# infancy/ky

Measured on AMD Instinct MI355X. Metric: Msamples/s (paths*spp), higher is better.
Workload: dtype f32

## Files before the change

### include/kyhip.h

```cpp
#ifndef KYHIP_H
#define KYHIP_H

#ifndef __HIPCC_RTC__
#include <stddef.h>
#include <stdint.h>
#endif

#ifdef __cplusplus
extern "C" {
#endif

#define KYHIP_ABI_VERSION 4


typedef enum ky_shape_kind {
    KY_SHAPE_DISK      = 0,
    KY_SHAPE_TRIANGLE  = 1,
    KY_SHAPE_RECTANGLE = 2,
    KY_SHAPE_SPHERE    = 3
} ky_shape_kind;

typedef struct ky_shape {
    int32_t kind;
    float   p[4][3];
// ... 102 lines not shown
    int32_t  tile_first, tile_step;
} ky_render_params;

typedef enum ky_status {
    KY_OK                = 0,
    KY_ERR_INVALID_VALUE = -1,
    KY_ERR_LIMIT         = -2,
    KY_ERR_DEVICE        = -3,
    KY_ERR_NO_DEVICE     = -4
} ky_status;

const char* kyhip_last_error(void);
int         kyhip_set_engine(int engine);
int         kyhip_set_specialisation(int on);
int         kyhip_set_boxes(int on);
int         kyhip_set_shadow_queue(int mode);
int         kyhip_set_jit(int mode);
const char* kyhip_jit_status(void);
int         kyhip_jit_failures(void);
int64_t     kyhip_jit_compile(const char* name_expression);
uint64_t    kyhip_kernel_source_hash(void);
int         kyhip_abi_version(void);
int         kyhip_device_count(void);

int64_t kyhip_shard_tile_count(const ky_render_params* params);
int64_t kyhip_shard_float_count(const ky_render_params* params);
int64_t kyhip_film_term_limit(const ky_render_params* params, int n_lights, int engine, int deferred, float* limit);

int kyhip_render(int device, const ky_scene* scene, const ky_render_params* params,
                 float* film_rgb, size_t film_row_stride_px);
// ... 61 lines not shown

int kyhip_kat_intersect(int device, const ky_shape* shape, const float* rays7, int n, float* out8);

int kyhip_kat_camera(int device, const ky_camera* camera, const float* p_film2, int n, float* out6);

int kyhip_kat_bsdf(int device, const ky_material* material, const float* in12, int n, float* out13);

int kyhip_kat_light(int device, const ky_scene* scene, int light, const float* in11, int n, float* out11);

int kyhip_kat_scene_intersect(int device, const ky_scene* scene, const float* rays7, int n, float* out9);
int kyhip_kat_occluded(int device, const ky_scene* scene, const float* in9, int n, float* out1);
int kyhip_kat_any_pair(int device, const ky_scene* scene, const float* in13, int n, float* out2);
int kyhip_kat_occluded_between(int device, const ky_scene* scene, int light, const float* in9, int n, float* out1);
int kyhip_scene_non_occluders(const ky_scene* scene, int light, int* left_out, int n);
int kyhip_scene_boxes(const ky_scene* scene, int* box_face, int n);
int kyhip_scene_facts(const ky_scene* scene);

int kyhip_kat_li(int device, const ky_scene* scene, const ky_render_params* params,
                 int x, int y, int s0, int n, float* out3);

int kyhip_kat_nee(int device, const ky_scene* scene, int direct_sample, int light, const float* in15, int n, float* out6);
int kyhip_kat_single_light(int device, const ky_scene* scene, const float* in16, int n, float* out6);

int kyhip_kat_li_trace(int device, const ky_scene* scene, const ky_render_params* params, int x, int y, int s,
                       float* rows26, int max_rows, float* li3);

enum ky_smallpt_refl { KY_SP_DIFF = 0, KY_SP_SPEC = 1, KY_SP_REFR = 2 };

typedef struct ky_smallpt_sphere {
    double rad;
// ... 29 lines not shown
```

### ky_amd/_abi.py

```python
import ctypes as C
import os

_HERE = os.path.dirname(os.path.abspath(__file__))
LIB_DIR = os.path.join(_HERE, "lib")
REPO_ROOT = os.path.dirname(_HERE)

SHAPE_DISK, SHAPE_TRIANGLE, SHAPE_RECTANGLE, SHAPE_SPHERE = 0, 1, 2, 3
MATERIAL_MATTE, MATERIAL_MIRROR, MATERIAL_GLASS, MATERIAL_PLASTIC = 0, 1, 2, 3
LIGHT_POINT, LIGHT_DIRECTION, LIGHT_AREA, LIGHT_ENVIRONMENT = 0, 1, 2, 3
INTEGRATOR_POSITION, INTEGRATOR_NORMAL, INTEGRATOR_BASECOLOR = 0, 1, 2
INTEGRATOR_DIRECT_LIGHTING, INTEGRATOR_PATH_TRACING_ITERATION = 6, 11
INTEGRATOR_SIMPLE_PATH_TRACING_RECURSION, INTEGRATOR_PATH_TRACING_RECURSION, INTEGRATOR_PATH_TRACING_RECURSION_DEFERED = 8, 9, 10
DIRECT_IDLE, DIRECT_BSDF, DIRECT_LIGHT, DIRECT_BSDF_MIS, DIRECT_LIGHT_MIS, DIRECT_BOTH_MIS = 0, 4, 8, 16, 32, 48
DIRECT_SINGLE_LIGHT, DIRECT_SINGLE_BOTH_MIS = 1, 49
SAMPLER_DEBUG, SAMPLER_RANDOM = 0, 1
LIGHTING_EMIT, LIGHTING_DIRECT, LIGHTING_INDIRECT, LIGHTING_ALL = 1, 2, 4, 7
SP_VARIANT_SMALLPT, SP_VARIANT_REWRITE = 0, 1
KY_OK, KY_ERR_INVALID_VALUE, KY_ERR_LIMIT, KY_ERR_DEVICE, KY_ERR_NO_DEVICE = 0, -1, -2, -3, -4
MAX_SHAPES, MAX_SURFACES, MAX_MATERIALS, MAX_LIGHTS = 256, 256, 64, 16

CB_LIGHT_AREA, CB_LIGHT_DIRECTION, CB_LIGHT_POINT, CB_LIGHT_ENVIRONMENT = 1, 2, 4, 8
CB_LARGE_MIRROR, CB_LARGE_GLASS, CB_SMALL_MIRROR, CB_SMALL_GLASS = 16, 32, 64, 128
CB_BOTH_SMALL_SPHERES = CB_SMALL_MIRROR | CB_SMALL_GLASS
CB_DEFAULT_SCENE = CB_BOTH_SMALL_SPHERES | CB_LIGHT_AREA
# ... 58 lines not shown

class SmallptParams(C.Structure):
    _fields_ = [("width", C.c_int), ("height", C.c_int), ("samps", C.c_int), ("seed", C.c_uint32), ("max_depth", C.c_int),
                ("variant", C.c_int)]


SP_DIFF, SP_SPEC, SP_REFR = 0, 1, 2
SSP = C.POINTER(SmallptSphere)
SPP = C.POINTER(SmallptParams)

KYHIP_SYMBOLS = {
    "kyhip_last_error": (C.c_char_p, []),
    "kyhip_set_engine": (C.c_int, [C.c_int]),
    "kyhip_set_specialisation": (C.c_int, [C.c_int]),
    "kyhip_set_boxes": (C.c_int, [C.c_int]),
    "kyhip_set_shadow_queue": (C.c_int, [C.c_int]),
    "kyhip_set_jit": (C.c_int, [C.c_int]),
    "kyhip_jit_status": (C.c_char_p, []),
    "kyhip_jit_failures": (C.c_int, []),
    "kyhip_multi_status": (C.c_char_p, [C.c_int]),
    "kyhip_film_alloc": (C.c_void_p, [C.c_size_t]),
    "kyhip_film_free": (None, [C.c_void_p]),
    "kyhip_seam_threads": (C.c_int, []),
    "kyhip_jit_compile": (C.c_int64, [C.c_char_p]),
    "kyhip_kernel_source_hash": (C.c_uint64, []),
    "kyhip_abi_version": (C.c_int, []),
    "kyhip_device_count": (C.c_int, []),
    "kyhip_shard_tile_count": (C.c_int64, [PP]),
    "kyhip_shard_float_count": (C.c_int64, [PP]),
    "kyhip_film_term_limit": (C.c_int64, [PP, C.c_int, C.c_int, C.c_int, C.POINTER(C.c_float)]),
# ... 35 lines not shown
    "kyhip_kat_li_trace": (C.c_int, [C.c_int, SP, PP, C.c_int, C.c_int, C.c_int, C.c_void_p, C.c_int, C.c_void_p]),
    "kyhip_smallpt_scene": (C.c_int, [SSP]),
    "kyhip_smallpt_scene_rewrite": (C.c_int, [SSP]),
    "kyhip_smallpt_render": (C.c_int, [C.c_int, SSP, C.c_int, SPP, C.c_void_p]),
    "kyhip_smallpt_kat_radiance": (C.c_int, [C.c_int, SSP, C.c_int, SPP, C.c_int, C.c_int, C.c_int, C.c_int, C.c_int, C.c_int, C.c_void_p]),
    "kyhip_kat_intersect": (C.c_int, [C.c_int, C.POINTER(Shape), C.c_void_p, C.c_int, C.c_void_p]),
    "kyhip_kat_camera": (C.c_int, [C.c_int, C.POINTER(Camera), C.c_void_p, C.c_int, C.c_void_p]),
    "kyhip_kat_bsdf": (C.c_int, [C.c_int, C.POINTER(Material), C.c_void_p, C.c_int, C.c_void_p]),
    "kyhip_kat_light": (C.c_int, [C.c_int, SP, C.c_int, C.c_void_p, C.c_int, C.c_void_p]),
    "kyhip_kat_scene_intersect": (C.c_int, [C.c_int, SP, C.c_void_p, C.c_int, C.c_void_p]),
    "kyhip_kat_occluded": (C.c_int, [C.c_int, SP, C.c_void_p, C.c_int, C.c_void_p]),
    "kyhip_kat_any_pair": (C.c_int, [C.c_int, SP, C.c_void_p, C.c_int, C.c_void_p]),
    "kyhip_kat_occluded_between": (C.c_int, [C.c_int, SP, C.c_int, C.c_void_p, C.c_int, C.c_void_p]),
    "kyhip_scene_non_occluders": (C.c_int, [SP, C.c_int, C.c_void_p, C.c_int]),
    "kyhip_scene_boxes": (C.c_int, [SP, C.c_void_p, C.c_int]),
    "kyhip_scene_facts": (C.c_int, [SP]),
    "kyhip_kat_li": (C.c_int, [C.c_int, SP, PP, C.c_int, C.c_int, C.c_int, C.c_int, C.c_void_p]),
}

KYHOST_SYMBOLS = {
    "kyhost_last_error": (C.c_char_p, []),
    "kyhost_scene_create_cornell_box": (C.c_void_p, [C.c_int, C.c_float, C.c_float]),
    "kyhost_scene_create_mis": (C.c_void_p, [C.c_float, C.c_float]),
    "kyhost_scene_destroy": (None, [C.c_void_p]),
    "kyhost_scene_flatten": (SP, [C.c_void_p]),
    "kyhost_render": (C.c_int, [C.c_void_p, C.c_int, C.c_int, C.c_int, C.c_int, C.c_int, C.c_uint, C.c_int, C.c_int,
                                C.c_int, C.c_int, C.c_int, C.c_void_p, C.c_int]),
    "kyhost_render_lighting": (C.c_int, [C.c_void_p, C.c_int, C.c_int, C.c_int, C.c_int, C.c_int, C.c_uint, C.c_int, C.c_int,
                                         C.c_int, C.c_int, C.c_int, C.c_void_p, C.c_int, C.c_int]),
    "kyhost_debug_area": (C.c_int, [C.c_void_p, C.c_int, C.c_int, C.c_int, C.c_int, C.c_int, C.c_uint, C.c_int, C.c_int,
# ... 101 lines not shown
```

### ky_amd/api.py

```python
import ctypes as C

import numpy as np

from . import _abi as A


class KyError(RuntimeError):
    pass


def _check(rc, lib=None):
    if rc != A.KY_OK:
        lib = lib or A.load_kyhip()
        raise KyError(f"kyhip error {rc}: {lib.kyhip_last_error().decode()}")


def _fptr(a):
    assert a.dtype == np.float32 and a.flags["C_CONTIGUOUS"]
    return a.ctypes.data_as(C.c_void_p)


class SceneHandle:

    def __init__(self, ptr):
# ... 382 lines not shown
    if rc < 0:
        _check(rc)
    return rc


def scene_boxes(scene):
    lib = A.load_kyhip()
    n = _scene_ptr(scene).contents.surface_count
    out = np.zeros(max(1, n), np.int32)
    rc = lib.kyhip_scene_boxes(_scene_ptr(scene), out.ctypes.data_as(C.c_void_p), n)
    if rc < 0:
        _check(rc)
    return rc, out[:n].copy()


def kat_li(scene, params, x, y, s0, n, device=0):
    lib = A.load_kyhip()
    out = np.zeros((n, 3), np.float32)
    _check(lib.kyhip_kat_li(device, _scene_ptr(scene), C.byref(params), x, y, s0, n, _fptr(out)))
    return out


def kat_li_lighting(scene, params, lighting, x, y, s0, n, device=0):
    lib = A.load_kyhip()
    out = np.zeros((n, 3), np.float32)
    _check(lib.kyhip_kat_li_lighting(device, _scene_ptr(scene), C.byref(params), int(lighting), x, y, s0, n, _fptr(out)))
    return out


def kat_nee(scene, direct_sample, light, in15, device=0):
# ... 66 lines not shown
```

### ky_amd/csrc/ky_host.hpp

```cpp
#pragma once
#include <cstddef>
#include <cstdint>
#include <condition_variable>
#include <functional>
#include <mutex>
#include <string>
#include <utility>
#include <vector>
#include <sys/types.h>

#include "ky_shard.hpp"

namespace kyh {
using namespace kyd;

int fail(int code, const char* fmt, ...) __attribute__((format(printf, 2, 3)));
const std::string& last_error();

bool valid_params(const ky_render_params* p);
bool shard_in_range(const ky_render_params* p);
ShardConst make_shard(const ky_render_params* p);
RenderConst make_rc(const ky_render_params* p);
long long film_term_count(const ky_render_params* p, int n_lights, bool queue_engine, bool deferred);
float film_term_limit(long long n_terms);
// ... 29 lines not shown
struct NonOccluders {
    std::vector<char> wall;
    std::vector<char> light_ok;
    bool deferred_ok = false;
    int ts_light = -1;
    double ts_plane[4] = {0, 0, 0, 0};
    std::vector<char> ts_behind;
};
void find_non_occluders(const ky_scene* in, NonOccluders& R);
struct Boxes {
    struct Box { float lo[3], hi[3]; int face[6]; };
    std::vector<Box> box;
    std::vector<int> box_of;
};
void find_boxes(const ky_scene* in, Boxes& B);
int pack_scene(const ky_scene* in, DScene* out);
uint64_t scene_hash(const DScene& s);
bool scene_input(const ky_scene* in, std::vector<unsigned char>& out, uint64_t& hash);

constexpr int KY_SP_MAX_SPHERES = 32;
int smallpt_check(const ky_smallpt_sphere* spheres, int n, const ky_smallpt_params* p);

bool specialisation_enabled();
bool boxes_enabled();
int shadow_queue_mode();
bool shadow_queue_wanted(const ky_scene* scene);
int blocks_per_cu_cap();
enum { KY_ENGINE_LANE = 0, KY_ENGINE_QUEUE = 1 };
int current_engine();

int cpus_granted();
int seam_threads();
void host_add_rows(float* __restrict__ film, size_t stride_px, const float* __restrict__ src, int width, int y0, int y1);
class HostPool {
public:
    void run(int n, const std::function<void(int)>& fn);
private:
    void loop(int id);
    std::mutex job_m_, m_;
// ... 27 lines not shown
```

### ky_amd/csrc/ky_hostcheck.cpp

```cpp
#include <atomic>
#include <cstdlib>
#include <cstring>
#include <memory>
#include <thread>
#include <sys/wait.h>
#include <unistd.h>

#include "ky_blocks.hpp"
#include "ky_host.hpp"
#include "ky_noise.hpp"

using namespace kyh;

extern "C" {

int kyhostcheck_pack(const ky_scene* scene, int* feat, uint64_t* packed_hash, uint64_t* input_hash, int* n_planar_occ, int* ts_light) {
    std::unique_ptr<DScene> d(new DScene);
    const int rc = pack_scene(scene, d.get());
    if (rc != KY_OK) return rc;
    if (feat) *feat = d->feat;
    if (packed_hash) *packed_hash = scene_hash(*d);
    std::vector<unsigned char> in;
    uint64_t h = 0;
    const bool keyed = scene_input(scene, in, h);
// ... 178 lines not shown
        if (init) s = inside > 0 ? BlockState{-1, 0} : BlockState{0, 0};
        if (map && s.retired_at < 0) {
            int counted = 0, above = 0;
            for (int lane = 0; lane < KY_BLOCK_PIXELS; ++lane) {
                const int i = pixel_of_block(sh, b, lane);
                const int c = cls ? cls[i] : (pixel_inside(sh, i, p->width, p->height) ? kyn::KY_NOISE_INSIDE : kyn::KY_NOISE_PADDING);
                counted += c == kyn::KY_NOISE_INSIDE;
                above += c == kyn::KY_NOISE_INSIDE && map[i] > threshold;
            }
            if (block_retires(batches, min_batches, above, counted, max_fraction_above)) s = BlockState{front, batches};
        }
        state[2 * b] = s.retired_at; state[2 * b + 1] = s.batches;
    }
    if (!trailer) return KY_OK;
    return block_trailer_check(trailer, trailer_bytes, trailer_offset, sh.n_blocks, p->samples_per_pixel, samples_done, noise_batches);
}

static int no_gpu() { return fail(KY_ERR_NO_DEVICE, "sanitizer build of the host-only code: no GPU entry points"); }
int kyhip_device_count(void) { return 0; }
int kyhip_render(int, const ky_scene*, const ky_render_params* p, float*, size_t) { return valid_params(p) ? no_gpu() : fail(KY_ERR_INVALID_VALUE, "invalid render params"); }
int kyhip_render_multi(const int*, int, const ky_scene*, const ky_render_params* p, float*, size_t) { return valid_params(p) ? no_gpu() : fail(KY_ERR_INVALID_VALUE, "invalid render params"); }
int kyhip_render_tiles_device(int, const ky_scene*, const ky_render_params* p, float*, void*, size_t, void*) { return valid_params(p) ? no_gpu() : fail(KY_ERR_INVALID_VALUE, "invalid render params"); }
int kyhip_film_add_tiles_device(int, const ky_render_params*, const float*, float*, size_t, void*) { return no_gpu(); }
int kyhip_film_add_gathered_device(int, const ky_render_params*, int, const float*, size_t, float*, size_t, void*) { return no_gpu(); }
float kyhip_kernel_ms(int) { return -1.f; }
const char* kyhip_last_kernel(int) { return ""; }
const char* kyhip_multi_status(int) { return ""; }
void* kyhip_film_alloc(size_t) { return nullptr; }
void kyhip_film_free(void*) {}
int kyhip_kat_intersect(int, const ky_shape*, const float*, int, float*) { return no_gpu(); }
// ... 77 lines not shown
```

### ky_amd/csrc/ky_pack.cpp

```cpp
#include <algorithm>
#include <cmath>
#include <cstdarg>
#include <cstdio>
#include <cstdlib>
#include <cstring>
#include <limits>
#include <thread>
#include <sched.h>
#include <unistd.h>

#include "ky_blocks.hpp"
#include "ky_host.hpp"
#include "ky_noise.hpp"

namespace kyh {

static thread_local std::string g_error;

int fail(int code, const char* fmt, ...) {
    char buf[512];
    va_list ap;
    va_start(ap, fmt);
    vsnprintf(buf, sizeof buf, fmt, ap);
    va_end(ap);
// ... 523 lines not shown
        const char* e = std::getenv("KYHIP_SPECIALISE");
        g_specialise = (e && std::atoi(e) == 0) ? 0 : 1;
    }
    return g_specialise != 0;
}

static int g_boxes = -1;
bool boxes_enabled() {
    if (g_boxes < 0) {
        const char* e = std::getenv("KYHIP_BOXES");
        g_boxes = (e && std::atoi(e) == 0) ? 0 : 1;
    }
    return g_boxes != 0;
}

int pack_scene(const ky_scene* in, DScene* out) {
    if (!in) return fail(KY_ERR_INVALID_VALUE, "scene is NULL");
    if (in->surface_count < 0 || in->shape_count < 0 || in->material_count < 0 || in->light_count < 0)
        return fail(KY_ERR_INVALID_VALUE, "negative count in scene");
    if (in->surface_count > KYHIP_MAX_SURFACES || in->shape_count > KYHIP_MAX_SHAPES || in->material_count > KYHIP_MAX_MATERIALS ||
        in->light_count > KYHIP_MAX_LIGHTS)
        return fail(KY_ERR_LIMIT, "scene exceeds device limits (%d surfaces, %d shapes, %d materials, %d lights)", in->surface_count,
                    in->shape_count, in->material_count, in->light_count);
    if (in->environment_light < -1 || in->environment_light >= in->light_count) return fail(KY_ERR_INVALID_VALUE, "environment_light out of range");
    std::memset(out, 0, sizeof *out);
    out->n_surfaces = in->surface_count; out->n_lights = in->light_count; out->n_materials = in->material_count;
    out->env_light = in->environment_light;
    cp3(out->cam_position, in->camera.position); cp3(out->cam_front, in->camera.front); cp3(out->cam_right, in->camera.right);
    cp3(out->cam_up, in->camera.up);
    out->cam_inv_w = 1.f / in->camera.resolution[0]; out->cam_inv_h = 1.f / in->camera.resolution[1];
// ... 87 lines not shown
            }
            if (!fits) continue;
            DBox& d = BT.box[BT.n_box++];
            d.q0 = make_float4(b.lo[0], b.lo[1], b.lo[2], 0.f);
            d.q1 = make_float4(b.hi[0], b.hi[1], b.hi[2], 0.f);
            std::memcpy(&d.q0.w, &tag[0], 4); std::memcpy(&d.q1.w, &tag[1], 4);
            std::memcpy(&d.q2.x, &tag[2], 4); std::memcpy(&d.q2.y, &tag[3], 4); std::memcpy(&d.q2.z, &tag[4], 4); std::memcpy(&d.q2.w, &tag[5], 4);
            for (int f = 0; f < 6; ++f) if (b.face[f] >= 0) boxed[b.face[f]] = 1;
        }
        for (const PlanarEntry& e : planar)
            if (e.axis >= 0 && !boxed[e.surface]) { BT.n_aar_axis[e.axis]++; BT.aar[BT.n_aar++] = e.aar; }
        if (BT.n_aar > 0) BT.aar[BT.n_aar] = BT.aar[BT.n_aar - 1];
    }
    out->occ_deferred_ok = non.deferred_ok ? 1 : 0;
    out->ts_light = non.ts_light;
    out->feat = 0;
    if (specialisation_enabled()) {
        if (in->light_count == 1 && in->lights[0].kind == KY_LIGHT_AREA && in->environment_light < 0) out->feat |= KY_FEAT_SINGLE_AREA;
        if (in->light_count == 1 && (in->lights[0].kind == KY_LIGHT_POINT || in->lights[0].kind == KY_LIGHT_DIRECTION) && in->environment_light < 0)
            out->feat |= KY_FEAT_SINGLE_DELTA;
        if (in->light_count == 1 && in->lights[0].kind == KY_LIGHT_ENVIRONMENT && in->environment_light == 0) out->feat |= KY_FEAT_SINGLE_ENV;
        bool rect = true;
        for (int i = 0; i < in->light_count; ++i)
            if (in->lights[i].kind == KY_LIGHT_AREA) rect = rect && in->shapes[in->lights[i].shape].kind == KY_SHAPE_RECTANGLE;
        if (rect) out->feat |= KY_FEAT_RECT_LIGHTS;
        bool spheres = in->light_count > 0 && in->environment_light < 0;
        for (int i = 0; i < in->light_count; ++i)
            spheres = spheres && in->lights[i].kind == KY_LIGHT_AREA && in->shapes[in->lights[i].shape].kind == KY_SHAPE_SPHERE;
        for (int i = 0; i < in->surface_count; ++i)
            if (in->surfaces[i].area_light >= 0) spheres = spheres && in->shapes[in->surfaces[i].shape].kind == KY_SHAPE_SPHERE;
// ... 134 lines not shown
    uint64_t h0 = 0x9E3779B97F4A7C15ull, h1 = 0xC2B2AE3D27D4EB4Full;
    for (size_t i = 0; i + 1 < sizeof(DScene) / 8; i += 2) {
        h0 = (h0 ^ w[i]) * 0xff51afd7ed558ccdull; h0 ^= h0 >> 29;
        h1 = (h1 ^ w[i + 1]) * 0xc4ceb9fe1a85ec53ull; h1 ^= h1 >> 31;
    }
    if ((sizeof(DScene) / 8) & 1) h0 = (h0 ^ w[sizeof(DScene) / 8 - 1]) * 0xff51afd7ed558ccdull;
    return h0 ^ (h1 * 0x9E3779B97F4A7C15ull);
}

bool scene_input(const ky_scene* in, std::vector<unsigned char>& out, uint64_t& hash) {
    out.clear();
    if (!in || in->surface_count < 0 || in->shape_count < 0 || in->material_count < 0 || in->light_count < 0 || in->surface_count > KYHIP_MAX_SURFACES ||
        in->shape_count > KYHIP_MAX_SHAPES || in->material_count > KYHIP_MAX_MATERIALS || in->light_count > KYHIP_MAX_LIGHTS)
        return false;
    auto put = [&](const void* p, size_t n) { const unsigned char* b = (const unsigned char*)p; out.insert(out.end(), b, b + n); };
    const int32_t head[6] = {in->shape_count, in->material_count, in->light_count, in->surface_count, in->environment_light, (specialisation_enabled() ? 1 : 0) | (boxes_enabled() ? 2 : 0)};
    put(head, sizeof head);
    put(&in->camera, sizeof in->camera);
    if (in->shape_count) put(in->shapes, sizeof(ky_shape) * (size_t)in->shape_count);
    if (in->material_count) put(in->materials, sizeof(ky_material) * (size_t)in->material_count);
    if (in->light_count) put(in->lights, sizeof(ky_light) * (size_t)in->light_count);
    if (in->surface_count) put(in->surfaces, sizeof(ky_surface) * (size_t)in->surface_count);
    out.resize((out.size() + 7) & ~(size_t)7, 0);
    uint64_t h = 0x9E3779B97F4A7C15ull;
    for (size_t i = 0; i < out.size(); i += 8) {
        uint64_t w;
        std::memcpy(&w, &out[i], 8);
        h = (h ^ w) * 0xff51afd7ed558ccdull;
        h ^= h >> 29;
    }
    hash = h;
// ... 79 lines not shown

int smallpt_check(const ky_smallpt_sphere* spheres, int n, const ky_smallpt_params* p) {
    if (!spheres || !p) return fail(KY_ERR_INVALID_VALUE, "null argument");
    if (p->variant != KY_SP_VARIANT_SMALLPT && p->variant != KY_SP_VARIANT_REWRITE) return fail(KY_ERR_INVALID_VALUE, "unknown smallpt variant %d", p->variant);
    if (n <= 0 || n > KY_SP_MAX_SPHERES) return fail(KY_ERR_INVALID_VALUE, "1..%d spheres", KY_SP_MAX_SPHERES);
    if (p->width <= 0 || p->height <= 0 || p->width > 16384 || p->height > 16384 || p->samps <= 0 || p->max_depth < 0)
        return fail(KY_ERR_INVALID_VALUE, "invalid smallpt params");
    for (int i = 0; i < n; ++i)
        if (spheres[i].refl < KY_SP_DIFF || spheres[i].refl > KY_SP_REFR || !(spheres[i].rad > 0)) return fail(KY_ERR_INVALID_VALUE, "sphere %d is invalid", i);
    return KY_OK;
}

void set_engine_raw(int v) { g_engine = v; }
void set_specialise_raw(int v) { g_specialise = v; }
void set_boxes_raw(int v) { g_boxes = v; }
void set_shadow_queue_raw(int v) { g_shadow_queue = v; }
}

using namespace kyh;

extern "C" {

const char* kyhip_last_error(void) { return kyh::last_error().c_str(); }
int kyhip_seam_threads(void) { return kyh::seam_threads(); }
int kyhip_abi_version(void) { return KYHIP_ABI_VERSION; }


int kyhip_set_engine(int engine) {
    const int prev = current_engine();
    if (engine == KY_ENGINE_LANE || engine == KY_ENGINE_QUEUE) kyh::set_engine_raw(engine);
    return prev;
}
int kyhip_set_specialisation(int on) {
    const int prev = specialisation_enabled() ? 1 : 0;
    if (on == 0 || on == 1) kyh::set_specialise_raw(on);
    return prev;
}
int kyhip_set_boxes(int on) {
    const int prev = boxes_enabled() ? 1 : 0;
    if (on == 0 || on == 1) kyh::set_boxes_raw(on);
    return prev;
}
int kyhip_set_shadow_queue(int mode) {
    const int prev = shadow_queue_mode();
    if (mode >= -1 && mode <= 1) kyh::set_shadow_queue_raw(mode);
    return prev;
}

int kyhip_lighting_check(int integrator, int lighting) { return lighting_check(integrator, lighting); }
int kyhip_lighting_plan(const ky_render_params* p, int lighting, int* effective_depth, int* dropped) {
    LightingPlan pl;
    const int rc = lighting_plan(p, lighting, &pl);
    if (rc != KY_OK) return rc;
    if (effective_depth) *effective_depth = pl.effective_depth;
    if (dropped) *dropped = pl.dropped;
// ... 60 lines not shown
    const int rc = pack_scene(scene, &packed[0]);
    if (rc != KY_OK) return rc;
    if (n < scene->surface_count) return fail(KY_ERR_INVALID_VALUE, "box_face holds %d entries, the scene has %d surfaces", n, scene->surface_count);
    for (int i = 0; i < scene->surface_count; ++i) box_face[i] = -1;
    const DScene& P = packed[0];
    for (int b = 0; b < P.boxtrav.n_box; ++b) {
        const DBox& d = P.boxtrav.box[b];
        const float* src[6] = {&d.q0.w, &d.q1.w, &d.q2.x, &d.q2.y, &d.q2.z, &d.q2.w};
        for (int f = 0; f < 6; ++f) {
            uint32_t sidx;
            std::memcpy(&sidx, src[f], 4);
            if (sidx != (uint32_t)KY_BOX_NO_FACE) box_face[P.orig[sidx]] = 8 * b + f;
        }
    }
    return P.boxtrav.n_box;
}

int kyhip_smallpt_scene(ky_smallpt_sphere* out) {
    if (!out) return fail(KY_ERR_INVALID_VALUE, "null output");
    struct Row { double rad, p[3], e[3], c[3]; int refl; };
    static const Row rows[9] = {
        {1e5, {1e5 + 1, 40.8, 81.6}, {0, 0, 0}, {.75, .25, .25}, KY_SP_DIFF},
        {1e5, {-1e5 + 99, 40.8, 81.6}, {0, 0, 0}, {.25, .25, .75}, KY_SP_DIFF},
        {1e5, {50, 40.8, 1e5}, {0, 0, 0}, {.75, .75, .75}, KY_SP_DIFF},
        {1e5, {50, 40.8, -1e5 + 170}, {0, 0, 0}, {0, 0, 0}, KY_SP_DIFF},
        {1e5, {50, 1e5, 81.6}, {0, 0, 0}, {.75, .75, .75}, KY_SP_DIFF},
        {1e5, {50, -1e5 + 81.6, 81.6}, {0, 0, 0}, {.75, .75, .75}, KY_SP_DIFF},
        {16.5, {27, 16.5, 47}, {0, 0, 0}, {1 * .999, 1 * .999, 1 * .999}, KY_SP_SPEC},
        {16.5, {73, 16.5, 78}, {0, 0, 0}, {1 * .999, 1 * .999, 1 * .999}, KY_SP_REFR},
        {600, {50, 681.6 - .27, 81.6}, {12, 12, 12}, {0, 0, 0}, KY_SP_DIFF}};
// ... 19 lines not shown
```

### ky_amd/csrc/ky_render.hpp

```cpp
#pragma once
#include "ky_device.hpp"
#include "ky_shard.hpp"

using namespace kyd;

#ifndef KY_MAX_RETRACE
#define KY_MAX_RETRACE 1
#endif
#ifndef KY_REFILL_BATCH
#define KY_REFILL_BATCH 6
#endif
#ifndef KY_REFILL_WAIT
#define KY_REFILL_WAIT 4
#endif
#ifndef KY_RETRACE_THRESHOLD
#define KY_RETRACE_THRESHOLD 80
#endif
#ifndef KY_WAVES_PER_EU
#define KY_WAVES_PER_EU 7
#endif
#ifndef KY_WAVES_PER_EU_QUEUE
#define KY_WAVES_PER_EU_QUEUE 6
#endif
#ifndef KY_WAVES_PER_EU_QUEUE_FEAT
// ... 119 lines not shown
            const int n_need = __popcll(need_mask);
            while (!exhausted && cursor + n_need > fetched * 64) {
                unsigned id = blockIdx.x * 4u + (threadIdx.x >> 6);
                if (fetched > 0 && lane == 0) id = atomicAdd(counter, 1u) + gridDim.x * 4u;
                id = __builtin_amdgcn_readfirstlane(id);
                if (id >= sh.n_items) { exhausted = true; break; }
                const int c = (int)(id / (unsigned)sh.n_blocks) + sh.chunk_first;
                int b = (int)(id % (unsigned)sh.n_blocks);
                if constexpr (LISTED) {
                    typedef const int __attribute__((address_space(4))) * LiveList;
                    b = __builtin_amdgcn_readfirstlane(((LiveList)(const int*)(flags + sh.n_pix))[b]);
                }
                const int k = b / sh.blocks_per_tile, inner = b % sh.blocks_per_tile;
                const int bx = inner % sh.blocks_w, by = inner / sh.blocks_w;
                const int tile = sh.tile_first + k * sh.tile_step;
                if (lane == 0) {
                    ItemSlot it;
                    const int trow = tile / sh.tiles_x, tcol = (tile % sh.tiles_x + trow) % sh.tiles_x;
                    it.x0 = tcol * sh.tile_w + bx * 8;
                    it.y0 = trow * sh.tile_h + by * 8;
                    it.pix0 = (k * sh.tile_h + by * 8) * sh.tile_w + bx * 8;
                    chunk_range(chunk_plan(rc.spp), c, it.s_begin, it.s_end);
                    my_ring[fetched % KY_RING] = it;
                }
                ++fetched;
            }
            __builtin_amdgcn_fence(__ATOMIC_ACQ_REL, "wavefront");
            if (need) {
                const int mine = cursor + (int)__builtin_amdgcn_mbcnt_hi((unsigned)(need_mask >> 32), __builtin_amdgcn_mbcnt_lo((unsigned)need_mask, 0u));
                if (mine < fetched * 64) {
                    const ItemSlot it = my_ring[(mine >> 6) % KY_RING];
                    const int px = mine & 7, py = (mine >> 3) & 7;
                    const int x = it.x0 + px, y = it.y0 + py;
                    const bool in_range = x < rc.width && y < rc.height;
                    c_xy[tid] = x | (y << 16);
                    c_pix[tid] = it.pix0 + py * sh.tile_w + px;
                    if (!QUEUE) c_key[tid] = sampler_pixel_key(rc.seed, (uint32_t)(y * rc.width + x));
                    c_se[tid] = ((unsigned)it.s_begin << 7) | (unsigned)(it.s_end - it.s_begin);
// ... 79 lines not shown
```

### ky_amd/csrc/ky_scene.hpp

```cpp
#pragma once
#ifndef __HIPCC_RTC__
#include <hip/hip_vector_types.h>
#include <stdint.h>
#endif

#include "../../include/kyhip.h"

#if defined(__HIPCC__) || defined(__HIPCC_RTC__)
#define KY_HD __host__ __device__
#else
#define KY_HD
#endif

namespace kyd {

enum : int {
    TK_DISK = KY_SHAPE_DISK,
    TK_TRIANGLE = KY_SHAPE_TRIANGLE,
    TK_QUAD = KY_SHAPE_RECTANGLE,
    TK_SPHERE = KY_SHAPE_SPHERE,
    TK_PARALLELOGRAM = 4
};

struct DSurf {
// ... 47 lines not shown
    float e1[3];
    float inv_area;
    float n[3];
    int32_t n_carriers;
    int32_t carrier[4];
    int32_t sampled_is_surface;
    int32_t occ_ok;
    int32_t pdf_from_carrier;
    int32_t shadow_table;
    float aar[5];
    int32_t aar_axis;
    int32_t pad_a[2];
    DSurf isect;
};
constexpr int KY_MAX_CARRIERS = 4;
static_assert(sizeof(DLight) % 16 == 0 && __builtin_offsetof(DLight, p1) % 16 == 0 && __builtin_offsetof(DLight, n) % 16 == 0, "DLight is read in 16-byte groups (shape_sample_position)");

struct DPar {
    float4 q0, q1, q2;
};
struct DSph {
    float4 c;
};
struct DAar {
    float4 q0, q1;
};

struct DBox {
    float4 q0, q1, q2;
};
// ... 10 lines not shown
    int32_t n_aar_axis[3], pad_t2;
    DAar aar[KYHIP_MAX_SURFACES + 1];
    DPar par[KYHIP_MAX_SURFACES + 1];
};
struct DScene {
    int32_t n_surfaces, n_lights, n_materials, env_light;
    int32_t n_sph, n_gen, general, occ_deferred_ok;
    float cam_position[3], cam_inv_w;
    float cam_front[3], cam_inv_h;
    float cam_right[3], pad0;
    float cam_up[3], pad1;
    DTrav trav;
    DTrav occ;
    int32_t ts_light, feat, ts_pad[2];
    float ts_plane[4];
    DTrav occ_front, occ_behind;
    DBoxTrav boxtrav;
    DSph sph[KYHIP_MAX_SURFACES + 1];
    DSurf gen[KYHIP_MAX_SURFACES];
    DSurf all[KYHIP_MAX_SURFACES];
    DShapeFull full[KYHIP_MAX_SURFACES + KYHIP_MAX_LIGHTS];
    DHit hit[KYHIP_MAX_SURFACES];
    int32_t orig[KYHIP_MAX_SURFACES];
    DMat mat[KYHIP_MAX_MATERIALS];
    DLight light[KYHIP_MAX_LIGHTS];
};
static_assert(__builtin_offsetof(DScene, light) % 16 == 0 && __builtin_offsetof(DScene, trav) % 16 == 0 && __builtin_offsetof(DScene, boxtrav) % 16 == 0 &&
              __builtin_offsetof(DBoxTrav, box) % 16 == 0, "16-byte scalar loads of light, table and box records");


// ... 32 lines not shown
```

Measured before the change: 22160.

## Skip 8x8 pixel blocks whose screen area cannot see any scene geometry

On the host, the scene's world bounding box is projected through the camera into a conservative screen rectangle of live pixels, which is stored in the packed scene. In the persistent render loop, each 8x8 block is tested against that rectangle and skipped if it lies wholly outside, since with no environment light such pixels would only gather zero radiance. The culling is turned off whenever a bound is unsafe: an environment light, non-finite geometry, or geometry behind or straddling the camera. Each fetched block now pays one extra scene read and a wave-uniform branch, and a Cornell-box-style view where the camera sits inside or near the geometry will usually cull nothing.

```diff
diff --git a/include/kyhip.h b/include/kyhip.h
--- a/include/kyhip.h
+++ b/include/kyhip.h
@@ -140,6 +140,7 @@
 int         kyhip_set_engine(int engine);
 int         kyhip_set_specialisation(int on);
 int         kyhip_set_boxes(int on);
+int         kyhip_set_screen_cull(int on);
 int         kyhip_set_shadow_queue(int mode);
 int         kyhip_set_jit(int mode);
 const char* kyhip_jit_status(void);
@@ -231,6 +232,7 @@
 int kyhip_kat_occluded_between(int device, const ky_scene* scene, int light, const float* in9, int n, float* out1);
 int kyhip_scene_non_occluders(const ky_scene* scene, int light, int* left_out, int n);
 int kyhip_scene_boxes(const ky_scene* scene, int* box_face, int n);
+int kyhip_scene_screen_bound(const ky_scene* scene, const ky_render_params* params, int rect[4], long long counts[2]);
 int kyhip_scene_facts(const ky_scene* scene);
 
 int kyhip_kat_li(int device, const ky_scene* scene, const ky_render_params* params,
diff --git a/ky_amd/_abi.py b/ky_amd/_abi.py
--- a/ky_amd/_abi.py
+++ b/ky_amd/_abi.py
@@ -96,6 +96,7 @@
     "kyhip_set_engine": (C.c_int, [C.c_int]),
     "kyhip_set_specialisation": (C.c_int, [C.c_int]),
     "kyhip_set_boxes": (C.c_int, [C.c_int]),
+    "kyhip_set_screen_cull": (C.c_int, [C.c_int]),
     "kyhip_set_shadow_queue": (C.c_int, [C.c_int]),
     "kyhip_set_jit": (C.c_int, [C.c_int]),
     "kyhip_jit_status": (C.c_char_p, []),
@@ -161,6 +162,7 @@
     "kyhip_kat_occluded_between": (C.c_int, [C.c_int, SP, C.c_int, C.c_void_p, C.c_int, C.c_void_p]),
     "kyhip_scene_non_occluders": (C.c_int, [SP, C.c_int, C.c_void_p, C.c_int]),
     "kyhip_scene_boxes": (C.c_int, [SP, C.c_void_p, C.c_int]),
+    "kyhip_scene_screen_bound": (C.c_int, [SP, PP, C.POINTER(C.c_int), C.POINTER(C.c_longlong)]),
     "kyhip_scene_facts": (C.c_int, [SP]),
     "kyhip_kat_li": (C.c_int, [C.c_int, SP, PP, C.c_int, C.c_int, C.c_int, C.c_int, C.c_void_p]),
 }
diff --git a/ky_amd/api.py b/ky_amd/api.py
--- a/ky_amd/api.py
+++ b/ky_amd/api.py
@@ -420,6 +420,14 @@
     return rc, out[:n].copy()
 
 
+def scene_screen_bound(scene, params):
+    lib = A.load_kyhip()
+    rect = (C.c_int * 4)()
+    counts = (C.c_longlong * 2)()
+    _check(lib.kyhip_scene_screen_bound(_scene_ptr(scene), C.byref(params), rect, counts))
+    return tuple(int(v) for v in rect), int(counts[0]), int(counts[1])
+
+
 def kat_li(scene, params, x, y, s0, n, device=0):
     lib = A.load_kyhip()
     out = np.zeros((n, 3), np.float32)
diff --git a/ky_amd/csrc/ky_host.hpp b/ky_amd/csrc/ky_host.hpp
--- a/ky_amd/csrc/ky_host.hpp
+++ b/ky_amd/csrc/ky_host.hpp
@@ -67,6 +67,8 @@
     std::vector<int> box_of;
 };
 void find_boxes(const ky_scene* in, Boxes& B);
+void screen_bound(const ky_scene* in, int32_t live[4]);
+void screen_bound_counts(const int32_t live[4], const ky_render_params* p, long long* dead, long long* total);
 int pack_scene(const ky_scene* in, DScene* out);
 uint64_t scene_hash(const DScene& s);
 bool scene_input(const ky_scene* in, std::vector<unsigned char>& out, uint64_t& hash);
@@ -76,6 +78,7 @@
 
 bool specialisation_enabled();
 bool boxes_enabled();
+bool screen_cull_enabled();
 int shadow_queue_mode();
 bool shadow_queue_wanted(const ky_scene* scene);
 int blocks_per_cu_cap();
diff --git a/ky_amd/csrc/ky_hostcheck.cpp b/ky_amd/csrc/ky_hostcheck.cpp
--- a/ky_amd/csrc/ky_hostcheck.cpp
+++ b/ky_amd/csrc/ky_hostcheck.cpp
@@ -1,6 +1,7 @@
 #include <atomic>
 #include <cstdlib>
 #include <cstring>
+#include <limits>
 #include <memory>
 #include <thread>
 #include <sys/wait.h>
@@ -216,6 +217,84 @@
     }
     if (!trailer) return KY_OK;
     return block_trailer_check(trailer, trailer_bytes, trailer_offset, sh.n_blocks, p->samples_per_pixel, samples_done, noise_batches);
+}
+
+int kyhostcheck_screen_bound(void) {
+    const float q = std::numeric_limits<float>::quiet_NaN();
+    auto rect_shape = [](const float (&p)[4][3], float nx, float ny, float nz) {
+        ky_shape s{};
+        s.kind = KY_SHAPE_RECTANGLE;
+        std::memcpy(s.p, p, sizeof s.p);
+        s.normal[0] = nx; s.normal[1] = ny; s.normal[2] = nz;
+        return s;
+    };
+    const float back[4][3] = {{-1, -1, 1}, {1, -1, 1}, {1, 1, 1}, {-1, 1, 1}}, floor_[4][3] = {{-1, -1, -1}, {1, -1, -1}, {1, -1, 1}, {-1, -1, 1}},
+                ceil_[4][3] = {{-1, 1, -1}, {1, 1, -1}, {1, 1, 1}, {-1, 1, 1}}, left[4][3] = {{-1, -1, -1}, {-1, -1, 1}, {-1, 1, 1}, {-1, 1, -1}},
+                right[4][3] = {{1, -1, -1}, {1, -1, 1}, {1, 1, 1}, {1, 1, -1}};
+    std::vector<ky_shape> box = {rect_shape(back, 0, 0, -1), rect_shape(floor_, 0, 1, 0), rect_shape(ceil_, 0, -1, 0), rect_shape(left, 1, 0, 0), rect_shape(right, -1, 0, 0)};
+    ky_material matte{};
+    matte.kind = KY_MATERIAL_MATTE; matte.color0[0] = matte.color0[1] = matte.color0[2] = 0.5f;
+    ky_light lamp{};
+    lamp.kind = KY_LIGHT_POINT; lamp.color[0] = lamp.color[1] = lamp.color[2] = 1.f;
+    std::vector<ky_surface> surf;
+    for (int i = 0; i < 5; ++i) surf.push_back(ky_surface{i, 0, -1});
+    ky_render_params p{};
+    p.integrator = KY_INTEGRATOR_PATH_TRACING_ITERATION; p.max_path_depth = 5; p.direct_sample = KY_DIRECT_BOTH_MIS; p.samples_per_pixel = 4; p.sampler = KY_SAMPLER_RANDOM;
+    p.width = 256; p.height = 64; p.tile_w = 32; p.tile_h = 32; p.tile_first = 0; p.tile_step = 1;
+    auto scene_at = [&](const std::vector<ky_shape>& shapes, int n_surfaces, float cz) {
+        ky_scene s{};
+        s.shapes = shapes.data(); s.shape_count = (int)shapes.size();
+        s.materials = &matte; s.material_count = 1;
+        s.lights = &lamp; s.light_count = 1;
+        s.surfaces = surf.data(); s.surface_count = n_surfaces;
+        s.environment_light = -1;
+        s.camera.position[2] = cz; s.camera.front[2] = 1.f; s.camera.right[0] = 2.f; s.camera.up[1] = 0.5f;
+        s.camera.resolution[0] = 256.f; s.camera.resolution[1] = 64.f;
+        return s;
+    };
+    auto whole = [&](const ky_scene& s) {
+        int r[4] = {-1, -1, -1, -1};
+        long long c[2] = {-1, -1};
+        return kyhip_scene_screen_bound(&s, &p, r, c) == KY_OK && r[0] == 0 && r[1] == 0 && r[2] == p.width && r[3] == p.height && c[0] == 0 && c[1] == 8 * 32;
+    };
+    {
+        const ky_scene s = scene_at(box, 5, -5.f);
+        int r[4];
+        long long c[2];
+        if (kyhip_scene_screen_bound(&s, &p, r, c) != KY_OK || !(r[0] > 8 && r[2] < p.width - 8 && r[0] < 128 && r[2] > 128 && r[1] == 0 && r[3] == p.height && c[0] > 0 && c[0] < c[1])) return 1;
+    }
+    if (!whole(scene_at(box, 5, -1.f))) return 2;
+    if (!whole(scene_at(box, 5, 0.f))) return 3;
+    if (!whole(scene_at(box, 0, -5.f))) return 4;
+    {
+        std::vector<ky_shape> bad = box;
+        bad[2].p[1][0] = q;
+        if (!whole(scene_at(bad, 5, -5.f))) return 5;
+        bad = box;
+        bad[0].p[3][2] = std::numeric_limits<float>::infinity();
+        if (!whole(scene_at(bad, 5, -5.f))) return 6;
+    }
+    {
+        ky_shape sp{};
+        sp.kind = KY_SHAPE_SPHERE; sp.radius = 0.f;
+        std::vector<ky_shape> one = {sp};
+        const ky_scene s = scene_at(one, 1, -5.f);
+        int r[4];
+        if (kyhip_scene_screen_bound(&s, &p, r, nullptr) != KY_OK || !(r[0] >= 125 && r[0] <= 127 && r[2] >= 129 && r[2] <= 131 && r[1] >= 29 && r[3] <= 35)) return 7;
+        one[0].radius = q;
+        if (!whole(scene_at(one, 1, -5.f))) return 8;
+    }
+    {
+        const ky_scene s = scene_at(box, 5, -5.f);
+        const int prev = kyhip_set_screen_cull(0);
+        const bool off = whole(s);
+        kyhip_set_screen_cull(prev);
+        if (!off || kyhip_set_screen_cull(-1) != prev) return 9;
+        int32_t live[4];
+        screen_bound(nullptr, live);
+        if (live[0] != 0 || live[2] != KY_LIVE_MAX) return 10;
+    }
+    return 0;
 }
 
 static int no_gpu() { return fail(KY_ERR_NO_DEVICE, "sanitizer build of the host-only code: no GPU entry points"); }
diff --git a/ky_amd/csrc/ky_pack.cpp b/ky_amd/csrc/ky_pack.cpp
--- a/ky_amd/csrc/ky_pack.cpp
+++ b/ky_amd/csrc/ky_pack.cpp
@@ -561,6 +561,101 @@
     return g_boxes != 0;
 }
 
+static int g_screen_cull = -1;
+bool screen_cull_enabled() {
+    if (g_screen_cull < 0) {
+        const char* e = std::getenv("KYHIP_SCREEN_CULL");
+        g_screen_cull = (e && std::atoi(e) == 0) ? 0 : 1;
+    }
+    return g_screen_cull != 0;
+}
+
+void screen_bound(const ky_scene* in, int32_t live[4]) {
+    live[0] = live[1] = 0; live[2] = live[3] = KY_LIVE_MAX;
+    if (!in || !screen_cull_enabled() || in->environment_light >= 0 || in->surface_count <= 0 || !in->surfaces || !in->shapes) return;
+    double lo[3] = {0, 0, 0}, hi[3] = {0, 0, 0};
+    bool first = true;
+    auto add = [&](double x, double y, double z) {
+        const double v[3] = {x, y, z};
+        for (int k = 0; k < 3; ++k) { lo[k] = first ? v[k] : std::min(lo[k], v[k]); hi[k] = first ? v[k] : std::max(hi[k], v[k]); }
+        first = false;
+    };
+    for (int i = 0; i < in->surface_count; ++i) {
+        const int si = in->surfaces[i].shape;
+        if (si < 0 || si >= in->shape_count) return;
+        const ky_shape& sh = in->shapes[si];
+        if (sh.kind == KY_SHAPE_SPHERE || sh.kind == KY_SHAPE_DISK) {
+            const double r = std::fabs((double)sh.radius);
+            if (!std::isfinite(r) || !std::isfinite(sh.p[0][0]) || !std::isfinite(sh.p[0][1]) || !std::isfinite(sh.p[0][2])) return;
+            add(sh.p[0][0] - r, sh.p[0][1] - r, sh.p[0][2] - r);
+            add(sh.p[0][0] + r, sh.p[0][1] + r, sh.p[0][2] + r);
+        } else if (sh.kind == KY_SHAPE_TRIANGLE || sh.kind == KY_SHAPE_RECTANGLE) {
+            const int np = sh.kind == KY_SHAPE_TRIANGLE ? 3 : 4;
+            for (int q = 0; q < np; ++q) {
+                if (!std::isfinite(sh.p[q][0]) || !std::isfinite(sh.p[q][1]) || !std::isfinite(sh.p[q][2])) return;
+                add(sh.p[q][0], sh.p[q][1], sh.p[q][2]);
+            }
+        } else {
+            return;
+        }
+    }
+    const ky_camera& cam = in->camera;
+    double f[3], r[3], u[3], c[3];
+    for (int k = 0; k < 3; ++k) {
+        f[k] = cam.front[k]; r[k] = cam.right[k]; u[k] = cam.up[k]; c[k] = cam.position[k];
+        if (!std::isfinite(f[k]) || !std::isfinite(r[k]) || !std::isfinite(u[k]) || !std::isfinite(c[k])) return;
+    }
+    const double w = cam.resolution[0], h = cam.resolution[1];
+    if (!std::isfinite(w) || !std::isfinite(h) || !(w > 0) || !(h > 0)) return;
+    double diag = 0, size = 0;
+    for (int k = 0; k < 3; ++k) { diag += (hi[k] - lo[k]) * (hi[k] - lo[k]); size = std::max(size, std::max(std::fabs(lo[k]), std::fabs(hi[k]))); }
+    diag = std::sqrt(diag);
+    const double grow = std::max(1e-3 * diag, 1e-6 * size);
+    if (!std::isfinite(diag) || !std::isfinite(grow)) return;
+    auto cross3 = [](const double* x, const double* y, double* o) { o[0] = x[1] * y[2] - x[2] * y[1]; o[1] = x[2] * y[0] - x[0] * y[2]; o[2] = x[0] * y[1] - x[1] * y[0]; };
+    auto dot3 = [](const double* x, const double* y) { return x[0] * y[0] + x[1] * y[1] + x[2] * y[2]; };
+    double fs[3], rs[3], us[3];
+    cross3(r, u, fs); cross3(u, f, rs); cross3(f, r, us);
+    const double det = dot3(f, fs), lf = std::sqrt(dot3(f, f)), lr = std::sqrt(dot3(r, r)), lu = std::sqrt(dot3(u, u));
+    if (!std::isfinite(det) || !(std::fabs(det) > 1e-9 * lf * lr * lu) || !(lf > 0)) return;
+    double X0 = 0, X1 = 0, Y0 = 0, Y1 = 0;
+    int in_front = 0, behind = 0;
+    for (int corner = 0; corner < 8; ++corner) {
+        double v[3];
+        for (int k = 0; k < 3; ++k) v[k] = (((corner >> k) & 1) ? hi[k] + grow : lo[k] - grow) - c[k];
+        const double a = dot3(v, fs) / det, b = dot3(v, rs) / det, g = dot3(v, us) / det;
+        const double depth = a * lf, margin = std::max(grow, 1e-3 * diag);
+        if (!std::isfinite(depth)) return;
+        if (depth < -margin) { ++behind; continue; }
+        if (!(depth > margin)) return;
+        ++in_front;
+        const double x = (b / a + 0.5) * w, y = (0.5 - g / a) * h;
+        if (!std::isfinite(x) || !std::isfinite(y)) return;
+        X0 = in_front > 1 ? std::min(X0, x) : x; X1 = in_front > 1 ? std::max(X1, x) : x;
+        Y0 = in_front > 1 ? std::min(Y0, y) : y; Y1 = in_front > 1 ? std::max(Y1, y) : y;
+    }
+    if (behind == 8) { live[0] = live[1] = live[2] = live[3] = 0; return; }
+    if (in_front != 8) return;
+    auto clampi = [](double t) { return (int32_t)std::min((double)KY_LIVE_MAX, std::max(0.0, t)); };
+    live[0] = clampi(std::floor(X0) - 1); live[1] = clampi(std::floor(Y0) - 1);
+    live[2] = clampi(std::ceil(X1) + 1); live[3] = clampi(std::ceil(Y1) + 1);
+}
+
+void screen_bound_counts(const int32_t live[4], const ky_render_params* p, long long* dead, long long* total) {
+    const ShardConst sh = make_shard(p);
+    long long n_dead = 0;
+    for (int b = 0; b < sh.n_blocks; ++b) {
+        const int k = b / sh.blocks_per_tile, inner = b % sh.blocks_per_tile;
+        const int bx = inner % sh.blocks_w, by = inner / sh.blocks_w;
+        const int tile = sh.tile_first + k * sh.tile_step;
+        const int trow = tile / sh.tiles_x, tcol = (tile % sh.tiles_x + trow) % sh.tiles_x;
+        const int x0 = tcol * sh.tile_w + bx * 8, y0 = trow * sh.tile_h + by * 8;
+        n_dead += (x0 + 8 <= live[0] || x0 >= live[2] || y0 + 8 <= live[1] || y0 >= live[3]) ? 1 : 0;
+    }
+    if (dead) *dead = n_dead;
+    if (total) *total = sh.n_blocks;
+}
+
 int pack_scene(const ky_scene* in, DScene* out) {
     if (!in) return fail(KY_ERR_INVALID_VALUE, "scene is NULL");
     if (in->surface_count < 0 || in->shape_count < 0 || in->material_count < 0 || in->light_count < 0)
@@ -678,6 +773,7 @@
     }
     out->occ_deferred_ok = non.deferred_ok ? 1 : 0;
     out->ts_light = non.ts_light;
+    screen_bound(in, out->live);
     out->feat = 0;
     if (specialisation_enabled()) {
         if (in->light_count == 1 && in->lights[0].kind == KY_LIGHT_AREA && in->environment_light < 0) out->feat |= KY_FEAT_SINGLE_AREA;
@@ -842,7 +938,7 @@
         in->shape_count > KYHIP_MAX_SHAPES || in->material_count > KYHIP_MAX_MATERIALS || in->light_count > KYHIP_MAX_LIGHTS)
         return false;
     auto put = [&](const void* p, size_t n) { const unsigned char* b = (const unsigned char*)p; out.insert(out.end(), b, b + n); };
-    const int32_t head[6] = {in->shape_count, in->material_count, in->light_count, in->surface_count, in->environment_light, (specialisation_enabled() ? 1 : 0) | (boxes_enabled() ? 2 : 0)};
+    const int32_t head[6] = {in->shape_count, in->material_count, in->light_count, in->surface_count, in->environment_light, (specialisation_enabled() ? 1 : 0) | (boxes_enabled() ? 2 : 0) | (screen_cull_enabled() ? 4 : 0)};
     put(head, sizeof head);
     put(&in->camera, sizeof in->camera);
     if (in->shape_count) put(in->shapes, sizeof(ky_shape) * (size_t)in->shape_count);
@@ -952,6 +1048,7 @@
 void set_engine_raw(int v) { g_engine = v; }
 void set_specialise_raw(int v) { g_specialise = v; }
 void set_boxes_raw(int v) { g_boxes = v; }
+void set_screen_cull_raw(int v) { g_screen_cull = v; }
 void set_shadow_queue_raw(int v) { g_shadow_queue = v; }
 }
 
@@ -977,6 +1074,11 @@
 int kyhip_set_boxes(int on) {
     const int prev = boxes_enabled() ? 1 : 0;
     if (on == 0 || on == 1) kyh::set_boxes_raw(on);
+    return prev;
+}
+int kyhip_set_screen_cull(int on) {
+    const int prev = screen_cull_enabled() ? 1 : 0;
+    if (on == 0 || on == 1) kyh::set_screen_cull_raw(on);
     return prev;
 }
 int kyhip_set_shadow_queue(int mode) {
@@ -1067,6 +1169,20 @@
         }
     }
     return P.boxtrav.n_box;
+}
+
+int kyhip_scene_screen_bound(const ky_scene* scene, const ky_render_params* params, int rect[4], long long counts[2]) {
+    if (!scene || !rect) return fail(KY_ERR_INVALID_VALUE, "bad arguments");
+    if (!valid_params(params)) return fail(KY_ERR_INVALID_VALUE, "invalid render params");
+    if (!shard_in_range(params)) return fail(KY_ERR_LIMIT, "frame too large for the device's 32-bit work-item and pixel indices");
+    std::vector<DScene> packed(1);
+    const int rc = pack_scene(scene, &packed[0]);
+    if (rc != KY_OK) return rc;
+    const int32_t* live = packed[0].live;
+    rect[0] = std::min(live[0], params->width); rect[1] = std::min(live[1], params->height);
+    rect[2] = std::min(live[2], params->width); rect[3] = std::min(live[3], params->height);
+    if (counts) screen_bound_counts(live, params, &counts[0], &counts[1]);
+    return KY_OK;
 }
 
 int kyhip_smallpt_scene(ky_smallpt_sphere* out) {
diff --git a/ky_amd/csrc/ky_render.hpp b/ky_amd/csrc/ky_render.hpp
--- a/ky_amd/csrc/ky_render.hpp
+++ b/ky_amd/csrc/ky_render.hpp
@@ -157,14 +157,21 @@
                 const int k = b / sh.blocks_per_tile, inner = b % sh.blocks_per_tile;
                 const int bx = inner % sh.blocks_w, by = inner / sh.blocks_w;
                 const int tile = sh.tile_first + k * sh.tile_step;
+                int dead = 0;
                 if (lane == 0) {
                     ItemSlot it;
                     const int trow = tile / sh.tiles_x, tcol = (tile % sh.tiles_x + trow) % sh.tiles_x;
                     it.x0 = tcol * sh.tile_w + bx * 8;
                     it.y0 = trow * sh.tile_h + by * 8;
+                    const int4 live = scene_at<int4>(S, opaque_off((unsigned)__builtin_offsetof(DScene, live)));
+                    dead = (it.x0 + 8 <= live.x || it.x0 >= live.z || it.y0 + 8 <= live.y || it.y0 >= live.w) ? 1 : 0;
                     it.pix0 = (k * sh.tile_h + by * 8) * sh.tile_w + bx * 8;
                     chunk_range(chunk_plan(rc.spp), c, it.s_begin, it.s_end);
                     my_ring[fetched % KY_RING] = it;
+                }
+                if (__builtin_amdgcn_readfirstlane(dead)) {
+                    if (fetched == 0) { fetched = 1; cursor = 64; }
+                    continue;
                 }
                 ++fetched;
             }
diff --git a/ky_amd/csrc/ky_scene.hpp b/ky_amd/csrc/ky_scene.hpp
--- a/ky_amd/csrc/ky_scene.hpp
+++ b/ky_amd/csrc/ky_scene.hpp
@@ -85,6 +85,7 @@
     DSurf isect;
 };
 constexpr int KY_MAX_CARRIERS = 4;
+constexpr int KY_LIVE_MAX = 32768;
 static_assert(sizeof(DLight) % 16 == 0 && __builtin_offsetof(DLight, p1) % 16 == 0 && __builtin_offsetof(DLight, n) % 16 == 0, "DLight is read in 16-byte groups (shape_sample_position)");
 
 struct DPar {
@@ -125,6 +126,7 @@
     DTrav occ;
     int32_t ts_light, feat, ts_pad[2];
     float ts_plane[4];
+    int32_t live[4];
     DTrav occ_front, occ_behind;
     DBoxTrav boxtrav;
     DSph sph[KYHIP_MAX_SURFACES + 1];
```

Result: faster. 22960 (median of 6 runs) (+3.6%).
